# microsoft/AI2BMD

Hardware: NVIDIA H100
Metric: MD steps/sec (higher is better)
Workload: dtype f32

## Files before the change

ai2bmd_b200/csrc/common.cuh:

```cuda
#pragma once
#include <cuda_runtime.h>
#include <stdint.h>

namespace vb {

constexpr int D = 128;
constexpr int H = 8;
constexpr int NR = 32;
constexpr int L = 6;
constexpr int KNB = 32;
constexpr int LDS_PAD = 4;

__device__ __forceinline__ float sigmoidf_(float x) { return __fdividef(1.0f, 1.0f + __expf(-x)); }
__device__ __forceinline__ float silu_(float x) { return __fdividef(x, 1.0f + __expf(-x)); }
__device__ __forceinline__ float dsilu_(float x) {
    float s = sigmoidf_(x);
    return s * (1.0f + x * (1.0f - s));
}

__device__ __forceinline__ float4 ld4(const float* p) { return *reinterpret_cast<const float4*>(p); }
__device__ __forceinline__ float4 ldg4(const float* p) { return __ldg(reinterpret_cast<const float4*>(p)); }
__device__ __forceinline__ void st4(float* p, float4 v) { *reinterpret_cast<float4*>(p) = v; }
__device__ __forceinline__ void red4(float* p, float4 v) { atomicAdd(reinterpret_cast<float4*>(p), v); }

__device__ __forceinline__ float4 f4(float a, float b, float c, float d) { return make_float4(a, b, c, d); }
__device__ __forceinline__ float4 f4s(float a) { return make_float4(a, a, a, a); }
__device__ __forceinline__ float4 operator+(float4 a, float4 b) { return f4(a.x + b.x, a.y + b.y, a.z + b.z, a.w + b.w); }
__device__ __forceinline__ float4 operator-(float4 a, float4 b) { return f4(a.x - b.x, a.y - b.y, a.z - b.z, a.w - b.w); }
__device__ __forceinline__ float4 operator*(float4 a, float4 b) { return f4(a.x * b.x, a.y * b.y, a.z * b.z, a.w * b.w); }
__device__ __forceinline__ float4 operator*(float4 a, float b) { return f4(a.x * b, a.y * b, a.z * b, a.w * b); }
__device__ __forceinline__ float4 operator*(float b, float4 a) { return f4(a.x * b, a.y * b, a.z * b, a.w * b); }
__device__ __forceinline__ float hsum4(float4 a) { return (a.x + a.y) + (a.z + a.w); }
__device__ __forceinline__ float4 silu4(float4 a) { return f4(silu_(a.x), silu_(a.y), silu_(a.z), silu_(a.w)); }
__device__ __forceinline__ float4 dsilu4(float4 a) { return f4(dsilu_(a.x), dsilu_(a.y), dsilu_(a.z), dsilu_(a.w)); }
__device__ __forceinline__ float4 arr4(const float (&a)[4]) { return f4(a[0], a[1], a[2], a[3]); }

__device__ __forceinline__ float warp_sum(float v) {
#pragma unroll
    for (int o = 16; o > 0; o >>= 1) v += __shfl_xor_sync(0xffffffffu, v, o);
    return v;
}
__device__ __forceinline__ float warp_max(float v) {
#pragma unroll
    for (int o = 16; o > 0; o >>= 1) v = fmaxf(v, __shfl_xor_sync(0xffffffffu, v, o));
    return v;
}
__device__ __forceinline__ float warp_min(float v) {
#pragma unroll
    for (int o = 16; o > 0; o >>= 1) v = fminf(v, __shfl_xor_sync(0xffffffffu, v, o));
    return v;
}
__device__ __forceinline__ float quad_sum(float v) {
    v += __shfl_xor_sync(0xffffffffu, v, 1);
    v += __shfl_xor_sync(0xffffffffu, v, 2);
    return v;
}

template <int R>
__device__ __forceinline__ void warp_gemm_group(float (&acc)[R][4], const float* __restrict__ As, int lda, int k,
                                                const float4 (&w)[4]) {
#pragma unroll
    for (int r = 0; r < R; r++) {
        const float4 a = ld4(As + r * lda + k);
        acc[r][0] = fmaf(a.x, w[0].x, acc[r][0]); acc[r][1] = fmaf(a.x, w[0].y, acc[r][1]);
        acc[r][2] = fmaf(a.x, w[0].z, acc[r][2]); acc[r][3] = fmaf(a.x, w[0].w, acc[r][3]);
        acc[r][0] = fmaf(a.y, w[1].x, acc[r][0]); acc[r][1] = fmaf(a.y, w[1].y, acc[r][1]);
        acc[r][2] = fmaf(a.y, w[1].z, acc[r][2]); acc[r][3] = fmaf(a.y, w[1].w, acc[r][3]);
        acc[r][0] = fmaf(a.z, w[2].x, acc[r][0]); acc[r][1] = fmaf(a.z, w[2].y, acc[r][1]);
        acc[r][2] = fmaf(a.z, w[2].z, acc[r][2]); acc[r][3] = fmaf(a.z, w[2].w, acc[r][3]);
        acc[r][0] = fmaf(a.w, w[3].x, acc[r][0]); acc[r][1] = fmaf(a.w, w[3].y, acc[r][1]);
        acc[r][2] = fmaf(a.w, w[3].z, acc[r][2]); acc[r][3] = fmaf(a.w, w[3].w, acc[r][3]);
    }
}
__device__ __forceinline__ void warp_gemm_loadw(float4 (&w)[4], const float* __restrict__ Wp, int ldw, int k) {
    w[0] = ldg4(Wp + (size_t)(k + 0) * ldw);
    w[1] = ldg4(Wp + (size_t)(k + 1) * ldw);
    w[2] = ldg4(Wp + (size_t)(k + 2) * ldw);
    w[3] = ldg4(Wp + (size_t)(k + 3) * ldw);
}

template <int R, int K, int LDA, int NBUF = (R <= 4 ? 4 : 2)>
__device__ __forceinline__ void warp_gemm(float (&acc)[R][4], const float* __restrict__ As,
                                          const float* __restrict__ W, int ldw, int lane, int krot = 0) {
    static_assert(K % 16 == 0, "K must be a multiple of 16");
    const float* Wp = W + lane * 4;
    const auto kk = [&](int k) { return (k + krot) & (K - 1 | -(int)((K & (K - 1)) != 0)); };
    if constexpr (NBUF == 4) {
        float4 w0[4], w1[4], w2[4], w3[4];
        warp_gemm_loadw(w0, Wp, ldw, kk(0));
        warp_gemm_loadw(w1, Wp, ldw, kk(4));
        warp_gemm_loadw(w2, Wp, ldw, kk(8));
#pragma unroll 1
        for (int k = 0; k < K; k += 16) {
            warp_gemm_loadw(w3, Wp, ldw, kk(k + 12));
            warp_gemm_group<R>(acc, As, LDA, kk(k), w0);
            if (k + 16 < K) warp_gemm_loadw(w0, Wp, ldw, kk(k + 16));
            warp_gemm_group<R>(acc, As, LDA, kk(k + 4), w1);
            if (k + 16 < K) warp_gemm_loadw(w1, Wp, ldw, kk(k + 20));
            warp_gemm_group<R>(acc, As, LDA, kk(k + 8), w2);
            if (k + 16 < K) warp_gemm_loadw(w2, Wp, ldw, kk(k + 24));
            warp_gemm_group<R>(acc, As, LDA, kk(k + 12), w3);
        }
    } else {
        float4 w0[4], w1[4];
        warp_gemm_loadw(w0, Wp, ldw, kk(0));
#pragma unroll 1
        for (int k = 0; k < K; k += 8) {
            warp_gemm_loadw(w1, Wp, ldw, kk(k + 4));
            warp_gemm_group<R>(acc, As, LDA, kk(k), w0);
            if (k + 8 < K) warp_gemm_loadw(w0, Wp, ldw, kk(k + 8));
            warp_gemm_group<R>(acc, As, LDA, kk(k + 4), w1);
        }
    }
}

template <int K, int NPRE>
struct WarpGemmPre {
    static_assert((K & (K - 1)) == 0 && K % (4 * NPRE) == 0, "K: power of two and a multiple of the ring");
    float4 w[NPRE][4];
    const float* Wp;
    int ldw, krot;
    __device__ __forceinline__ int kk(int k) const { return (k + krot) & (K - 1); }
    __device__ __forceinline__ void prefetch(const float* __restrict__ W, int ldw_, int lane, int krot_) {
        Wp = W + lane * 4; ldw = ldw_; krot = krot_;
#pragma unroll
        for (int g = 0; g < NPRE; g++) warp_gemm_loadw(w[g], Wp, ldw, kk(4 * g));
    }
    template <int R, int LDA>
    __device__ __forceinline__ void run(float (&acc)[R][4], const float* __restrict__ As) {
#pragma unroll 1
        for (int k = 0; k < K; k += 4 * NPRE) {
#pragma unroll
            for (int g = 0; g < NPRE; g++) {
                warp_gemm_group<R>(acc, As, LDA, kk(k + 4 * g), w[g]);
                if (k + 4 * (g + NPRE) < K) warp_gemm_loadw(w[g], Wp, ldw, kk(k + 4 * (g + NPRE)));
            }
        }
    }
};

template <int R, int K, int LDA>
__device__ __forceinline__ void warp_gemm2(float (&acc)[R][2], const float* __restrict__ As,
                                           const float* __restrict__ W, int ldw, int lane) {
    const float* Wp = W + lane * 2;
#pragma unroll 4
    for (int k = 0; k < K; k += 4) {
        const float2 w0 = __ldg(reinterpret_cast<const float2*>(Wp + (size_t)(k + 0) * ldw));
        const float2 w1 = __ldg(reinterpret_cast<const float2*>(Wp + (size_t)(k + 1) * ldw));
        const float2 w2 = __ldg(reinterpret_cast<const float2*>(Wp + (size_t)(k + 2) * ldw));
        const float2 w3 = __ldg(reinterpret_cast<const float2*>(Wp + (size_t)(k + 3) * ldw));
#pragma unroll
        for (int r = 0; r < R; r++) {
            const float4 a = ld4(As + r * LDA + k);
            acc[r][0] = fmaf(a.x, w0.x, acc[r][0]); acc[r][1] = fmaf(a.x, w0.y, acc[r][1]);
            acc[r][0] = fmaf(a.y, w1.x, acc[r][0]); acc[r][1] = fmaf(a.y, w1.y, acc[r][1]);
            acc[r][0] = fmaf(a.z, w2.x, acc[r][0]); acc[r][1] = fmaf(a.z, w2.y, acc[r][1]);
            acc[r][0] = fmaf(a.w, w3.x, acc[r][0]); acc[r][1] = fmaf(a.w, w3.y, acc[r][1]);
        }
    }
}

template <int R>
__device__ __forceinline__ void acc_set_bias(float (&acc)[R][4], const float* __restrict__ b, int lane) {
    const float4 bb = ldg4(b + lane * 4);
#pragma unroll
    for (int r = 0; r < R; r++) { acc[r][0] = bb.x; acc[r][1] = bb.y; acc[r][2] = bb.z; acc[r][3] = bb.w; }
}
template <int R>
__device__ __forceinline__ void acc_zero(float (&acc)[R][4]) {
#pragma unroll
    for (int r = 0; r < R; r++) { acc[r][0] = 0.f; acc[r][1] = 0.f; acc[r][2] = 0.f; acc[r][3] = 0.f; }
}

__device__ __forceinline__ void pdl_entry() {
    asm volatile("griddepcontrol.wait;" ::: "memory");
}

__device__ __forceinline__ float cutoff_fn(float r, float rc) {
    return (r < rc) ? 0.5f * (cosf(r * (3.14159265358979323846f / rc)) + 1.0f) : 0.0f;
}
__device__ __forceinline__ float cutoff_dfn(float r, float rc) {
    const float w = 3.14159265358979323846f / rc;
    return (r < rc) ? -0.5f * w * sinf(r * w) : 0.0f;
}

}
```

ai2bmd_b200/csrc/k_node2.cuh:

```cuda
#pragma once
#include "k_node.cuh"

namespace vb {

template <int NB> struct N2Cfg {
    static constexpr int WARPS = (NB <= 4) ? 16 : 8; static constexpr int THREADS = WARPS * 32;
    static constexpr int KS = (NB <= 4) ? 2 : 1;
};
template <int NB> struct N2Rows { static constexpr int RB = (NB < 8) ? NB : 8; };

template <int NB>
struct NodeFwd2Smem {
    static constexpr int KS = N2Cfg<NB>::KS;
    static constexpr int LDA = D + LDS_PAD;
    static constexpr int LDO = 3 * D + LDS_PAD;
    float xs[NB][LDA];
    float vs[3 * NB][LDA];
    float os[NB][LDO];
    float osp[(NB <= 4) ? 3 : 1][NB][LDO];
    float px[(KS == 2) ? NB : 1][3 * D];
    float pv[(KS == 2) ? 3 * NB : 1][3 * D];
    float pt[(KS == 2) ? 3 * NB : 1][2 * D];
};

template <int NB>
__global__ void __launch_bounds__(N2Cfg<NB>::THREADS) node_fwd2_kernel(NodeArgs a) {
    pdl_entry();
    extern __shared__ __align__(16) float dyn_smem[];
    const ModelW& mw = a.mw;
    const Workspace& ws = a.ws;
    const int k = a.layer, n0 = (int)blockIdx.x * NB;
    unsigned long long* const tl = a.tl;
    const int krot = a.krot ? (int)blockIdx.x * 16 : 0;
#define N2_TL(i) do { if (tl != nullptr && n0 == 0 && (threadIdx.x & 31) == 0) tl[(i) * 16 + (threadIdx.x >> 5)] = (unsigned long long)clock64(); } while (0)
    N2_TL(0);
    constexpr int N2_WARPS = N2Cfg<NB>::WARPS, N2_THREADS = N2Cfg<NB>::THREADS, KS = N2Cfg<NB>::KS;
    using S = NodeFwd2Smem<NB>;
    constexpr int LDA = S::LDA;
    constexpr int N2_RB = N2Rows<NB>::RB;
    S& sm = *reinterpret_cast<S*>(dyn_smem);
    const int lane = threadIdx.x & 31, warp = threadIdx.x >> 5, col = lane * 4;
    const int nn = min(NB, ws.N - n0);

    if (k >= 1) {
        const LayerW& lw = mw.layer[k - 1];
        for (int idx = threadIdx.x; idx < NB * 32; idx += N2_THREADS) {
            const int nd = idx >> 5, c4 = (idx & 31) * 4;
            st4(&sm.xs[nd][c4], nd < nn ? ld4(ws.XA + (size_t)(n0 + nd) * D + c4) : f4s(0.f));
        }
        [[maybe_unused]] WarpGemmPre<D / 4, 4> go;
        if constexpr (KS == 2) {
            if (warp < 12) go.prefetch(lw.WoT + (size_t)(warp / 3) * (D / 4) * 3 * D + (warp % 3) * D, 3 * D, lane, krot);
        }
        __syncthreads();
        N2_TL(1);
        if constexpr (KS == 2) {
            if (warp < 12) {
                const int ch = warp % 3, kq = warp / 3;
                float acc[N2_RB][4];
                if (kq == 0) acc_set_bias<N2_RB>(acc, lw.bo + ch * D, lane);
                else acc_zero<N2_RB>(acc);
                go.template run<N2_RB, LDA>(acc, &sm.xs[0][kq * (D / 4)]);
#pragma unroll
                for (int r = 0; r < N2_RB; r++) {
                    if (kq == 0) st4(&sm.os[r][ch * D + col], arr4(acc[r]));
                    else st4(&sm.osp[kq - 1][r][ch * D + col], arr4(acc[r]));
                }
            }
            N2_TL(2);
            __syncthreads();
            N2_TL(3);
            for (int idx = threadIdx.x; idx < NB * 96; idx += N2_THREADS) {
                const int r = idx / 96, c4 = (idx % 96) * 4;
                st4(&sm.os[r][c4], (ld4(&sm.os[r][c4]) + ld4(&sm.osp[0][r][c4])) + (ld4(&sm.osp[1][r][c4]) + ld4(&sm.osp[2][r][c4])));
            }
        } else if constexpr (NB <= 4) {
            for (int u = warp; u < 12; u += N2_WARPS) {
                const int ch = u % 3, kq = u / 3;
                float acc[N2_RB][4];
                if (kq == 0) acc_set_bias<N2_RB>(acc, lw.bo + ch * D, lane);
                else acc_zero<N2_RB>(acc);
                warp_gemm<N2_RB, D / 4, LDA, 4>(acc, &sm.xs[0][kq * (D / 4)], lw.WoT + (size_t)kq * (D / 4) * 3 * D + ch * D, 3 * D, lane, krot);
#pragma unroll
                for (int r = 0; r < N2_RB; r++) {
                    if (kq == 0) st4(&sm.os[r][ch * D + col], arr4(acc[r]));
                    else st4(&sm.osp[kq - 1][r][ch * D + col], arr4(acc[r]));
                }
            }
            N2_TL(2);
            __syncthreads();
            N2_TL(3);
            for (int idx = threadIdx.x; idx < NB * 96; idx += N2_THREADS) {
                const int r = idx / 96, c4 = (idx % 96) * 4;
                st4(&sm.os[r][c4], (ld4(&sm.os[r][c4]) + ld4(&sm.osp[0][r][c4])) + (ld4(&sm.osp[1][r][c4]) + ld4(&sm.osp[2][r][c4])));
            }
        } else {
            for (int u = warp; u < 3 * (NB / N2_RB); u += N2_WARPS) {
                const int ch = u % 3, rb = u / 3;
                float acc[N2_RB][4];
                acc_set_bias<N2_RB>(acc, lw.bo + ch * D, lane);
                warp_gemm<N2_RB, D, LDA, (NB <= 8 ? 4 : 2)>(acc, &sm.xs[rb * N2_RB][0], lw.WoT + ch * D, 3 * D, lane);
#pragma unroll
                for (int r = 0; r < N2_RB; r++) st4(&sm.os[rb * N2_RB + r][ch * D + col], arr4(acc[r]));
            }
        }
        __syncthreads();
        N2_TL(4);
    }
    for (int nd = warp; nd < NB; nd += N2_WARPS) {
        const int node = n0 + nd;
        const bool ok = nd < nn;
        float4 x = f4s(0.f), vec[3] = {f4s(0.f), f4s(0.f), f4s(0.f)};
        if (k >= 1) {
            if (ok) {
                const float4 o1 = ld4(&sm.os[nd][col]), o2 = ld4(&sm.os[nd][D + col]), o3 = ld4(&sm.os[nd][2 * D + col]);
                float* orow = ws.O[k - 1] + (size_t)node * 3 * D;
                st4(orow + col, o1); st4(orow + D + col, o2); st4(orow + 2 * D + col, o3);
                x = ld4(ws.X[k - 1] + (size_t)node * D + col) + ld4(ws.VDOT[k - 1] + (size_t)node * D + col) * o2 + o3;
                st4(ws.X[k] + (size_t)node * D + col, x);
#pragma unroll
                for (int s = 0; s < 3; s++) {
                    const size_t r3 = (size_t)node * 3 + s;
                    vec[s] = ld4(ws.V[k - 1] + r3 * D + col) + ld4(ws.V123[k - 1] + r3 * 3 * D + 2 * D + col) * o1 +
                             ld4(ws.VA + r3 * D + col);
                    st4(ws.V[k] + r3 * D + col, vec[s]);
                }
            }
        } else if (ok) {
            x = ld4(ws.X[0] + (size_t)node * D + col);
        }
        if (ok) {
            st4(ws.XA + (size_t)node * D + col, f4s(0.f));
#pragma unroll
            for (int s = 0; s < 3; s++) st4(ws.VA + ((size_t)node * 3 + s) * D + col, f4s(0.f));
        }
        if (k < L) {
            const LayerW& lw = mw.layer[k];
            st4(&sm.xs[nd][col], ln_forward(x, lw.ln_w, lw.ln_b, lane));
            float4 vn[3];
            vecln_forward(vec, vn, lw.vln_w, lane);
#pragma unroll
            for (int s = 0; s < 3; s++) {
                st4(&sm.vs[nd * 3 + s][col], vn[s]);
                if (ok) st4(ws.VN[k] + ((size_t)node * 3 + s) * D + col, vn[s]);
            }
        }
    }
    N2_TL(5);
    if (k >= L) return;
    const LayerW& lw = mw.layer[k];
    constexpr int RV = 3 * NB, KH = D / 2;
    [[maybe_unused]] WarpGemmPre<KH, 2> gm;
    [[maybe_unused]] const int nunits2 = (k < L - 1) ? 16 : 12;
    [[maybe_unused]] const int kind = warp < 6 ? 0 : (warp < 12 ? 1 : 2);
    [[maybe_unused]] const int uv = kind == 0 ? warp : (kind == 1 ? warp - 6 : warp - 12);
    [[maybe_unused]] const int ch2 = kind == 2 ? (uv & 1) : uv % 3, half = kind == 2 ? (uv >> 1) : uv / 3;
    [[maybe_unused]] const bool active = warp < nunits2;
    if constexpr (KS == 2) {
        if (active) {
            const float* W = kind == 0 ? lw.WqkvT : (kind == 1 ? lw.WvecT : lw.WtuT);
            const int ldw = kind == 2 ? 2 * D : 3 * D;
            gm.prefetch(W + (size_t)half * KH * ldw + ch2 * D, ldw, lane, krot);
        }
    }
    __syncthreads();
    N2_TL(6);
    if constexpr (KS == 2) {
        const int ch = ch2;
        float acc[RV][4];
        float (&accx)[NB][4] = *reinterpret_cast<float (*)[NB][4]>(&acc[0][0]);
        if (active) {
            if (kind == 0) {
                if (half == 0) acc_set_bias<NB>(accx, lw.bqkv + ch * D, lane);
                else acc_zero<NB>(accx);
                gm.template run<NB, LDA>(accx, &sm.xs[0][half * KH]);
                if (half == 1) {
#pragma unroll
                    for (int r = 0; r < NB; r++) st4(&sm.px[r][ch * D + col], arr4(accx[r]));
                }
            } else {
                acc_zero<RV>(acc);
                gm.template run<RV, LDA>(acc, &sm.vs[0][half * KH]);
                if (half == 1) {
#pragma unroll
                    for (int r = 0; r < RV; r++) {
                        if (kind == 1) st4(&sm.pv[r][ch * D + col], arr4(acc[r]));
                        else           st4(&sm.pt[r][ch * D + col], arr4(acc[r]));
                    }
                }
            }
        }
        N2_TL(7);
        __syncthreads();
        N2_TL(8);
        if (active && half == 0) {
            if (kind == 0) {
#pragma unroll
                for (int r = 0; r < NB; r++)
                    if (r < nn) st4(ws.QKV[k] + (size_t)(n0 + r) * 3 * D + ch * D + col, arr4(accx[r]) + ld4(&sm.px[r][ch * D + col]));
            } else if (kind == 1) {
#pragma unroll
                for (int r = 0; r < RV; r++)
                    if (r / 3 < nn) st4(ws.V123[k] + ((size_t)n0 * 3 + r) * 3 * D + ch * D + col, arr4(acc[r]) + ld4(&sm.pv[r][ch * D + col]));
            } else {
#pragma unroll
                for (int r = 0; r < RV; r++)
                    if (r / 3 < nn) st4(ws.TU[k] + ((size_t)n0 * 3 + r) * 2 * D + ch * D + col, arr4(acc[r]) + ld4(&sm.pt[r][ch * D + col]));
            }
        }
    } else {
        constexpr int UQ = 3 * (NB / N2_RB), UV = 3 * (3 * NB / N2_RB), UT = 2 * (3 * NB / N2_RB);
        const int nunits = UQ + UV + ((k < L - 1) ? UT : 0);
        for (int u = warp; u < nunits; u += N2_WARPS) {
            float acc[N2_RB][4];
            if (u < UQ) {
                const int ch = u % 3, rb = u / 3;
                acc_set_bias<N2_RB>(acc, lw.bqkv + ch * D, lane);
                warp_gemm<N2_RB, D, LDA, (NB <= 8 ? 4 : 2)>(acc, &sm.xs[rb * N2_RB][0], lw.WqkvT + ch * D, 3 * D, lane);
    #pragma unroll
                for (int r = 0; r < N2_RB; r++) {
                    const int nd = rb * N2_RB + r;
                    if (nd < nn) st4(ws.QKV[k] + (size_t)(n0 + nd) * 3 * D + ch * D + col, arr4(acc[r]));
                }
            } else if (u < UQ + UV) {
                const int v = u - UQ, ch = v % 3, rb = v / 3;
                acc_zero<N2_RB>(acc);
                warp_gemm<N2_RB, D, LDA, (NB <= 8 ? 4 : 2)>(acc, &sm.vs[rb * N2_RB][0], lw.WvecT + ch * D, 3 * D, lane);
    #pragma unroll
                for (int r = 0; r < N2_RB; r++) {
                    const int row = rb * N2_RB + r;
                    if (row / 3 < nn) st4(ws.V123[k] + ((size_t)n0 * 3 + row) * 3 * D + ch * D + col, arr4(acc[r]));
                }
            } else {
                const int v = u - UQ - UV, ch = v % 2, rb = v / 2;
                acc_zero<N2_RB>(acc);
                warp_gemm<N2_RB, D, LDA, (NB <= 8 ? 4 : 2)>(acc, &sm.vs[rb * N2_RB][0], lw.WtuT + ch * D, 2 * D, lane);
    #pragma unroll
                for (int r = 0; r < N2_RB; r++) {
                    const int row = rb * N2_RB + r;
                    if (row / 3 < nn) st4(ws.TU[k] + ((size_t)n0 * 3 + row) * 2 * D + ch * D + col, arr4(acc[r]));
                }
            }
        }
    }
    N2_TL(9);
    __syncthreads();
    N2_TL(10);
    for (int nd = warp; nd < nn; nd += N2_WARPS) {
        const size_t r3 = (size_t)(n0 + nd) * 3;
        float4 vd = f4s(0.f);
#pragma unroll
        for (int s = 0; s < 3; s++) vd = vd + ld4(ws.V123[k] + (r3 + s) * 3 * D + col) * ld4(ws.V123[k] + (r3 + s) * 3 * D + D + col);
        st4(ws.VDOT[k] + (size_t)(n0 + nd) * D + col, vd);
    }
    N2_TL(11);
}

template <int NB>
struct NodeBwd2Smem {
    static constexpr int KS = N2Cfg<NB>::KS;
    static constexpr int LD3 = 3 * D + LDS_PAD;
    static constexpr int LD2 = 2 * D + LDS_PAD;
    static constexpr int NVB = 3 * NB / N2Rows<NB>::RB;
    static constexpr int NXB = NB / N2Rows<NB>::RB;
    float gq[NB][LD3];
    float gvp[3 * NB][LD3];
    float gtu[3 * NB][LD2];
    float part_x[3 * KS][NB][D];
    float part_v[5 * KS][3 * NB][D];
};

template <int NB>
__global__ void __launch_bounds__(N2Cfg<NB>::THREADS) node_bwd2_kernel(NodeArgs a) {
    pdl_entry();
    extern __shared__ __align__(16) float dyn_smem[];
    const ModelW& mw = a.mw;
    const Workspace& ws = a.ws;
    const int k = a.layer, n0 = (int)blockIdx.x * NB;
    unsigned long long* const tl = a.tl;
    const int krot = a.krot ? (int)blockIdx.x * 16 : 0;
    float* __restrict__ const GQKV = ws.GQKV;
    float* __restrict__ const GVNMSG = ws.GVNMSG;
    float* __restrict__ const GTU = ws.GTU;
    constexpr int N2_WARPS = N2Cfg<NB>::WARPS, KS = N2Cfg<NB>::KS;
    N2_TL(0);
    using S = NodeBwd2Smem<NB>;
    constexpr int LD3 = S::LD3, LD2 = S::LD2;
    constexpr int N2_RB = N2Rows<NB>::RB;
    S& sm = *reinterpret_cast<S*>(dyn_smem);
    const int lane = threadIdx.x & 31, warp = threadIdx.x >> 5, col = lane * 4;
    const int nn = min(NB, ws.N - n0);
    const bool has_a = (k <= L - 1), has_b = (k >= 1);
    const bool has_tu = (k < L - 1);
    const float4 z4 = f4s(0.f);

    if (has_a) {
        const LayerW& lw = mw.layer[k];
        for (int nd = warp; nd < NB; nd += N2_WARPS) {
            const int node = n0 + nd;
            const bool ok = nd < nn;
            const float4 gx = ok ? ld4(ws.GX + (size_t)node * D + col) : z4;
            const float* orow = ws.O[k] + (size_t)node * 3 * D;
            const float4 o1 = ok ? ld4(orow + col) : z4, o2 = ok ? ld4(orow + D + col) : z4;
            const float4 g_vdot = gx * o2;
            const float* gq = GQKV + (size_t)node * 3 * D;
            st4(&sm.gq[nd][col], ok ? ld4(gq + col) : z4);
            st4(&sm.gq[nd][D + col], ok ? ld4(gq + D + col) : z4);
            st4(&sm.gq[nd][2 * D + col], ok ? ld4(gq + 2 * D + col) : z4);
#pragma unroll
            for (int s = 0; s < 3; s++) {
                const size_t r3 = (size_t)node * 3 + s;
                const float* vrow = ws.V123[k] + r3 * 3 * D;
                const float4 gv = ok ? ld4(ws.GVEC + r3 * D + col) : z4;
                st4(&sm.gvp[nd * 3 + s][col], g_vdot * (ok ? ld4(vrow + D + col) : z4));
                st4(&sm.gvp[nd * 3 + s][D + col], g_vdot * (ok ? ld4(vrow + col) : z4));
                st4(&sm.gvp[nd * 3 + s][2 * D + col], gv * o1);
                if (has_tu) {
                    const float* gt = GTU + r3 * 2 * D;
                    st4(&sm.gtu[nd * 3 + s][col], ok ? ld4(gt + col) : z4);
                    st4(&sm.gtu[nd * 3 + s][D + col], ok ? ld4(gt + D + col) : z4);
                }
            }
        }
        constexpr int RV = 3 * NB, KH = D / 2;
        [[maybe_unused]] WarpGemmPre<KH, 2> gm;
        [[maybe_unused]] const int kv2 = has_tu ? 5 : 3;
        if constexpr (KS == 2) {
            const int u = warp;
            if (u < 6) gm.prefetch(lw.WqkvN + ((size_t)(u >> 1) * D + (u & 1) * KH) * D, D, lane, krot);
            else if (u < 6 + 2 * kv2) {
                const int v = u - 6, kc = v >> 1, hf = v & 1;
                gm.prefetch((kc < 3 ? lw.WvecN + (size_t)kc * D * D : lw.WtuN + (size_t)(kc - 3) * D * D) + (size_t)hf * KH * D, D, lane, krot);
            }
        }
        N2_TL(1);
        __syncthreads();
        N2_TL(2);
        if constexpr (KS == 2) {
            const int u = warp;
            if (u < 6) {
                const int kc = u >> 1, half = u & 1;
                float acc[NB][4];
                acc_zero<NB>(acc);
                gm.template run<NB, LD3>(acc, &sm.gq[0][kc * D + half * KH]);
#pragma unroll
                for (int r = 0; r < NB; r++) st4(&sm.part_x[u][r][col], arr4(acc[r]));
            } else if (u < 6 + 2 * kv2) {
                const int v = u - 6, kc = v >> 1, half = v & 1;
                float acc[RV][4];
                acc_zero<RV>(acc);
                if (kc < 3) gm.template run<RV, LD3>(acc, &sm.gvp[0][kc * D + half * KH]);
                else        gm.template run<RV, LD2>(acc, &sm.gtu[0][(kc - 3) * D + half * KH]);
#pragma unroll
                for (int r = 0; r < RV; r++) st4(&sm.part_v[v][r][col], arr4(acc[r]));
            }
        } else {
            constexpr int UX = 3 * S::NXB;
            const int kv = has_tu ? 5 : 3;
            const int nunits = UX + kv * S::NVB;
            for (int u = warp; u < nunits; u += N2_WARPS) {
                float acc[N2_RB][4];
                acc_zero<N2_RB>(acc);
                if (u < UX) {
                    const int kc = u % 3, rb = u / 3;
                    warp_gemm<N2_RB, D, LD3, 4>(acc, &sm.gq[rb * N2_RB][kc * D], lw.WqkvN + (size_t)kc * D * D, D, lane);
    #pragma unroll
                    for (int r = 0; r < N2_RB; r++) st4(&sm.part_x[kc][rb * N2_RB + r][col], arr4(acc[r]));
                } else {
                    const int v = u - UX, kc = v % kv, rb = v / kv;
                    if (kc < 3) warp_gemm<N2_RB, D, LD3, 4>(acc, &sm.gvp[rb * N2_RB][kc * D], lw.WvecN + (size_t)kc * D * D, D, lane);
                    else        warp_gemm<N2_RB, D, LD2, 4>(acc, &sm.gtu[rb * N2_RB][(kc - 3) * D], lw.WtuN + (size_t)(kc - 3) * D * D, D, lane);
    #pragma unroll
                    for (int r = 0; r < N2_RB; r++) st4(&sm.part_v[kc][rb * N2_RB + r][col], arr4(acc[r]));
                }
            }
        }
        N2_TL(3);
        __syncthreads();
        N2_TL(4);
    }
    for (int nd = warp; nd < NB; nd += N2_WARPS) {
        const int node = n0 + nd;
        const bool ok = nd < nn;
        float4 gx = ok ? ld4(ws.GX + (size_t)node * D + col) : z4, gvec[3];
#pragma unroll
        for (int s = 0; s < 3; s++) gvec[s] = ok ? ld4(ws.GVEC + ((size_t)node * 3 + s) * D + col) : z4;
        float4 v3p[3] = {z4, z4, z4}, vdp = z4;
        if (has_b && ok) {
#pragma unroll
            for (int s = 0; s < 3; s++) v3p[s] = ld4(ws.V123[k - 1] + ((size_t)node * 3 + s) * 3 * D + 2 * D + col);
            vdp = ld4(ws.VDOT[k - 1] + (size_t)node * D + col);
        }
        if (has_a && ok) {
            const LayerW& lw = mw.layer[k];
            const auto px = [&](int kc) {
                if constexpr (KS == 2) return ld4(&sm.part_x[2 * kc][nd][col]) + ld4(&sm.part_x[2 * kc + 1][nd][col]);
                else return ld4(&sm.part_x[kc][nd][col]);
            };
            const float4 gxn = (px(0) + px(1)) + px(2);
            float4 vin[3], gout[3], gv[3];
#pragma unroll
            for (int s = 0; s < 3; s++) {
                const int row = nd * 3 + s;
                const auto pv = [&](int kc) {
                    if constexpr (KS == 2) return ld4(&sm.part_v[2 * kc][row][col]) + ld4(&sm.part_v[2 * kc + 1][row][col]);
                    else return ld4(&sm.part_v[kc][row][col]);
                };
                float4 g = ld4(GVNMSG + ((size_t)node * 3 + s) * D + col);
                g = g + ((pv(0) + pv(1)) + pv(2));
                if (has_tu) g = g + (pv(3) + pv(4));
                gout[s] = g;
                vin[s] = ld4(ws.V[k] + ((size_t)node * 3 + s) * D + col);
            }
            vecln_backward(vin, gout, gv, lw.vln_w, lane);
#pragma unroll
            for (int s = 0; s < 3; s++) gvec[s] = gvec[s] + gv[s];
            gx = gx + ln_backward(ld4(ws.X[k] + (size_t)node * D + col), gxn, lw.ln_w, lane);
        }
        if (ok) {
            float* gq = GQKV + (size_t)node * 3 * D;
            st4(gq + col, z4); st4(gq + D + col, z4); st4(gq + 2 * D + col, z4);
#pragma unroll
            for (int s = 0; s < 3; s++) {
                const size_t r3 = (size_t)node * 3 + s;
                st4(GVNMSG + r3 * D + col, z4);
                st4(GTU + r3 * 2 * D + col, z4);
                st4(GTU + r3 * 2 * D + D + col, z4);
                st4(ws.GVEC + r3 * D + col, gvec[s]);
            }
            st4(ws.GX + (size_t)node * D + col, gx);
        }
        if (has_b) {
            float4 go1 = z4;
#pragma unroll
            for (int s = 0; s < 3; s++) go1 = go1 + gvec[s] * v3p[s];
            __syncwarp();
            st4(&sm.gq[nd][col], go1);
            st4(&sm.gq[nd][D + col], gx * vdp);
            st4(&sm.gq[nd][2 * D + col], gx);
        }
    }
    N2_TL(5);
    if (!has_b) return;
    const LayerW& lwo = mw.layer[k - 1];
    [[maybe_unused]] WarpGemmPre<D / 4, 4> go;
    if constexpr (KS == 2) {
        if (warp < 12) go.prefetch(lwo.WoN + ((size_t)(warp >> 2) * D + (warp & 3) * (D / 4)) * D, D, lane, krot);
    }
    __syncthreads();
    N2_TL(6);
    if constexpr (KS == 2) {
        float (*po)[NB][D] = reinterpret_cast<float (*)[NB][D]>(&sm.part_v[0][0][0]);
        if (warp < 12) {
            const int kc = warp >> 2, q = warp & 3;
            float acc[NB][4];
            acc_zero<NB>(acc);
            go.template run<NB, LD3>(acc, &sm.gq[0][kc * D + q * (D / 4)]);
#pragma unroll
            for (int r = 0; r < NB; r++) st4(&po[warp][r][col], arr4(acc[r]));
        }
        N2_TL(7);
        __syncthreads();
        N2_TL(8);
        for (int nd = warp; nd < nn; nd += N2_WARPS) {
            float4 t[3];
#pragma unroll
            for (int kc = 0; kc < 3; kc++)
                t[kc] = (ld4(&po[4 * kc][nd][col]) + ld4(&po[4 * kc + 1][nd][col])) + (ld4(&po[4 * kc + 2][nd][col]) + ld4(&po[4 * kc + 3][nd][col]));
            st4(ws.GXA + (size_t)(n0 + nd) * D + col, (t[0] + t[1]) + t[2]);
        }
        N2_TL(9);
    } else {
        for (int u = warp; u < 3 * S::NXB; u += N2_WARPS) {
            const int kc = u % 3, rb = u / 3;
            float acc[N2_RB][4];
            acc_zero<N2_RB>(acc);
            warp_gemm<N2_RB, D, LD3, 4>(acc, &sm.gq[rb * N2_RB][kc * D], lwo.WoN + (size_t)kc * D * D, D, lane);
#pragma unroll
            for (int r = 0; r < N2_RB; r++) st4(&sm.part_x[kc][rb * N2_RB + r][col], arr4(acc[r]));
        }
        __syncthreads();
        for (int nd = warp; nd < nn; nd += N2_WARPS)
            st4(ws.GXA + (size_t)(n0 + nd) * D + col,
                (ld4(&sm.part_x[0][nd][col]) + ld4(&sm.part_x[1][nd][col])) + ld4(&sm.part_x[2][nd][col]));
    }
}
#undef N2_TL

}
```

Measured before the change: 1154.

## Prefetch node glue inputs via cp.async and split scalar/vector glue across warps

The forward and backward node kernels now stage their per-node glue inputs (X, VDOT, V, V123, VA, GX, GVEC, GVNMSG and others) into shared memory with cp.async, issued before the weight prefetch and GEMMs. This hides global load latency behind other work. The glue loop is split so scalar and vector parts run on separate warps, and the partial-sum reduction of os/osp is folded into those warps, removing one block barrier. VDOT is computed from registers after a named barrier between two warps instead of re-reading V123 after a full sync. The cost is extra shared memory per block, which may lower occupancy, plus more complex synchronisation, and the NB<=4 path is removed.

```diff
diff --git a/ai2bmd_b200/csrc/common.cuh b/ai2bmd_b200/csrc/common.cuh
--- a/ai2bmd_b200/csrc/common.cuh
+++ b/ai2bmd_b200/csrc/common.cuh
@@ -22,6 +22,10 @@
 __device__ __forceinline__ float4 ldg4(const float* p) { return __ldg(reinterpret_cast<const float4*>(p)); }
 __device__ __forceinline__ void st4(float* p, float4 v) { *reinterpret_cast<float4*>(p) = v; }
 __device__ __forceinline__ void red4(float* p, float4 v) { atomicAdd(reinterpret_cast<float4*>(p), v); }
+__device__ __forceinline__ void cp4(float* s, const float* g) {
+    asm volatile("cp.async.cg.shared.global [%0], [%1], 16;" ::"r"((uint32_t)__cvta_generic_to_shared(s)), "l"(g) : "memory");
+}
+__device__ __forceinline__ void cp4_wait() { asm volatile("cp.async.wait_all;" ::: "memory"); }
 
 __device__ __forceinline__ float4 f4(float a, float b, float c, float d) { return make_float4(a, b, c, d); }
 __device__ __forceinline__ float4 f4s(float a) { return make_float4(a, a, a, a); }
diff --git a/ai2bmd_b200/csrc/k_node2.cuh b/ai2bmd_b200/csrc/k_node2.cuh
--- a/ai2bmd_b200/csrc/k_node2.cuh
+++ b/ai2bmd_b200/csrc/k_node2.cuh
@@ -18,6 +18,8 @@
     float vs[3 * NB][LDA];
     float os[NB][LDO];
     float osp[(NB <= 4) ? 3 : 1][NB][LDO];
+    float gl[(KS == 2) ? 11 * NB : 1][D];
+    float v1[(KS == 2) ? 3 * NB : 1][D];
     float px[(KS == 2) ? NB : 1][3 * D];
     float pv[(KS == 2) ? 3 * NB : 1][3 * D];
     float pt[(KS == 2) ? 3 * NB : 1][2 * D];
@@ -42,16 +44,35 @@
     const int lane = threadIdx.x & 31, warp = threadIdx.x >> 5, col = lane * 4;
     const int nn = min(NB, ws.N - n0);
 
+    [[maybe_unused]] const auto glue_in = [&](int row, const float* g) {
+        if constexpr (KS == 2) return ld4(&sm.gl[row][col]);
+        else return ld4(g + col);
+    };
     if (k >= 1) {
         const LayerW& lw = mw.layer[k - 1];
-        for (int idx = threadIdx.x; idx < NB * 32; idx += N2_THREADS) {
-            const int nd = idx >> 5, c4 = (idx & 31) * 4;
-            st4(&sm.xs[nd][c4], nd < nn ? ld4(ws.XA + (size_t)(n0 + nd) * D + c4) : f4s(0.f));
+        constexpr int NR = (KS == 2) ? 12 * NB : NB;
+        for (int idx = threadIdx.x; idx < NR * 32; idx += N2_THREADS) {
+            const int q = idx >> 5, c4 = (idx & 31) * 4;
+            const float* src;
+            int nd;
+            if (q < NB) { nd = q; src = ws.XA + (size_t)(n0 + nd) * D; }
+            else if (q < 2 * NB) { nd = q - NB; src = ws.X[k - 1] + (size_t)(n0 + nd) * D; }
+            else if (q < 3 * NB) { nd = q - 2 * NB; src = ws.VDOT[k - 1] + (size_t)(n0 + nd) * D; }
+            else {
+                const int r = (q - 3 * NB) % (3 * NB), part = (q - 3 * NB) / (3 * NB);
+                const size_t r3 = (size_t)n0 * 3 + r;
+                nd = r / 3;
+                src = part == 0 ? ws.V[k - 1] + r3 * D : (part == 1 ? ws.V123[k - 1] + r3 * 3 * D + 2 * D : ws.VA + r3 * D);
+            }
+            float* dst = q < NB ? &sm.xs[q][c4] : &sm.gl[q - NB][c4];
+            if (nd < nn) cp4(dst, src + c4);
+            else st4(dst, f4s(0.f));
         }
         [[maybe_unused]] WarpGemmPre<D / 4, 4> go;
         if constexpr (KS == 2) {
             if (warp < 12) go.prefetch(lw.WoT + (size_t)(warp / 3) * (D / 4) * 3 * D + (warp % 3) * D, 3 * D, lane, krot);
         }
+        cp4_wait();
         __syncthreads();
         N2_TL(1);
         if constexpr (KS == 2) {
@@ -67,33 +88,6 @@
                     else st4(&sm.osp[kq - 1][r][ch * D + col], arr4(acc[r]));
                 }
             }
-            N2_TL(2);
-            __syncthreads();
-            N2_TL(3);
-            for (int idx = threadIdx.x; idx < NB * 96; idx += N2_THREADS) {
-                const int r = idx / 96, c4 = (idx % 96) * 4;
-                st4(&sm.os[r][c4], (ld4(&sm.os[r][c4]) + ld4(&sm.osp[0][r][c4])) + (ld4(&sm.osp[1][r][c4]) + ld4(&sm.osp[2][r][c4])));
-            }
-        } else if constexpr (NB <= 4) {
-            for (int u = warp; u < 12; u += N2_WARPS) {
-                const int ch = u % 3, kq = u / 3;
-                float acc[N2_RB][4];
-                if (kq == 0) acc_set_bias<N2_RB>(acc, lw.bo + ch * D, lane);
-                else acc_zero<N2_RB>(acc);
-                warp_gemm<N2_RB, D / 4, LDA, 4>(acc, &sm.xs[0][kq * (D / 4)], lw.WoT + (size_t)kq * (D / 4) * 3 * D + ch * D, 3 * D, lane, krot);
-#pragma unroll
-                for (int r = 0; r < N2_RB; r++) {
-                    if (kq == 0) st4(&sm.os[r][ch * D + col], arr4(acc[r]));
-                    else st4(&sm.osp[kq - 1][r][ch * D + col], arr4(acc[r]));
-                }
-            }
-            N2_TL(2);
-            __syncthreads();
-            N2_TL(3);
-            for (int idx = threadIdx.x; idx < NB * 96; idx += N2_THREADS) {
-                const int r = idx / 96, c4 = (idx % 96) * 4;
-                st4(&sm.os[r][c4], (ld4(&sm.os[r][c4]) + ld4(&sm.osp[0][r][c4])) + (ld4(&sm.osp[1][r][c4]) + ld4(&sm.osp[2][r][c4])));
-            }
         } else {
             for (int u = warp; u < 3 * (NB / N2_RB); u += N2_WARPS) {
                 const int ch = u % 3, rb = u / 3;
@@ -104,51 +98,9 @@
                 for (int r = 0; r < N2_RB; r++) st4(&sm.os[rb * N2_RB + r][ch * D + col], arr4(acc[r]));
             }
         }
-        __syncthreads();
-        N2_TL(4);
-    }
-    for (int nd = warp; nd < NB; nd += N2_WARPS) {
-        const int node = n0 + nd;
-        const bool ok = nd < nn;
-        float4 x = f4s(0.f), vec[3] = {f4s(0.f), f4s(0.f), f4s(0.f)};
-        if (k >= 1) {
-            if (ok) {
-                const float4 o1 = ld4(&sm.os[nd][col]), o2 = ld4(&sm.os[nd][D + col]), o3 = ld4(&sm.os[nd][2 * D + col]);
-                float* orow = ws.O[k - 1] + (size_t)node * 3 * D;
-                st4(orow + col, o1); st4(orow + D + col, o2); st4(orow + 2 * D + col, o3);
-                x = ld4(ws.X[k - 1] + (size_t)node * D + col) + ld4(ws.VDOT[k - 1] + (size_t)node * D + col) * o2 + o3;
-                st4(ws.X[k] + (size_t)node * D + col, x);
-#pragma unroll
-                for (int s = 0; s < 3; s++) {
-                    const size_t r3 = (size_t)node * 3 + s;
-                    vec[s] = ld4(ws.V[k - 1] + r3 * D + col) + ld4(ws.V123[k - 1] + r3 * 3 * D + 2 * D + col) * o1 +
-                             ld4(ws.VA + r3 * D + col);
-                    st4(ws.V[k] + r3 * D + col, vec[s]);
-                }
-            }
-        } else if (ok) {
-            x = ld4(ws.X[0] + (size_t)node * D + col);
-        }
-        if (ok) {
-            st4(ws.XA + (size_t)node * D + col, f4s(0.f));
-#pragma unroll
-            for (int s = 0; s < 3; s++) st4(ws.VA + ((size_t)node * 3 + s) * D + col, f4s(0.f));
-        }
-        if (k < L) {
-            const LayerW& lw = mw.layer[k];
-            st4(&sm.xs[nd][col], ln_forward(x, lw.ln_w, lw.ln_b, lane));
-            float4 vn[3];
-            vecln_forward(vec, vn, lw.vln_w, lane);
-#pragma unroll
-            for (int s = 0; s < 3; s++) {
-                st4(&sm.vs[nd * 3 + s][col], vn[s]);
-                if (ok) st4(ws.VN[k] + ((size_t)node * 3 + s) * D + col, vn[s]);
-            }
-        }
-    }
-    N2_TL(5);
-    if (k >= L) return;
-    const LayerW& lw = mw.layer[k];
+        N2_TL(2);
+        __syncthreads();
+    }
     constexpr int RV = 3 * NB, KH = D / 2;
     [[maybe_unused]] WarpGemmPre<KH, 2> gm;
     [[maybe_unused]] const int nunits2 = (k < L - 1) ? 16 : 12;
@@ -156,12 +108,79 @@
     [[maybe_unused]] const int uv = kind == 0 ? warp : (kind == 1 ? warp - 6 : warp - 12);
     [[maybe_unused]] const int ch2 = kind == 2 ? (uv & 1) : uv % 3, half = kind == 2 ? (uv >> 1) : uv / 3;
     [[maybe_unused]] const bool active = warp < nunits2;
-    if constexpr (KS == 2) {
-        if (active) {
+    [[maybe_unused]] const auto prefetch_units = [&]() {
+        if (k < L && active) {
+            const LayerW& lw = mw.layer[k];
             const float* W = kind == 0 ? lw.WqkvT : (kind == 1 ? lw.WvecT : lw.WtuT);
             const int ldw = kind == 2 ? 2 * D : 3 * D;
             gm.prefetch(W + (size_t)half * KH * ldw + ch2 * D, ldw, lane, krot);
         }
+    };
+    if constexpr (KS == 2) {
+        if (warp >= 2 * NB) prefetch_units();
+    }
+    for (int it = warp; it < 2 * NB; it += N2_WARPS) {
+        const int nd = it % NB, node = n0 + nd;
+        const bool ok = nd < nn;
+        const auto o = [&](int c) {
+            if constexpr (KS == 2)
+                return (ld4(&sm.os[nd][c * D + col]) + ld4(&sm.osp[0][nd][c * D + col])) +
+                       (ld4(&sm.osp[1][nd][c * D + col]) + ld4(&sm.osp[2][nd][c * D + col]));
+            else return ld4(&sm.os[nd][c * D + col]);
+        };
+        if (it < NB) {
+            float4 x = f4s(0.f);
+            if (k >= 1) {
+                if (ok) {
+                    const float4 o2 = o(1), o3 = o(2);
+                    float* orow = ws.O[k - 1] + (size_t)node * 3 * D;
+                    st4(orow + D + col, o2); st4(orow + 2 * D + col, o3);
+                    x = glue_in(nd, ws.X[k - 1] + (size_t)node * D) + glue_in(NB + nd, ws.VDOT[k - 1] + (size_t)node * D) * o2 + o3;
+                    st4(ws.X[k] + (size_t)node * D + col, x);
+                }
+            } else if (ok) {
+                x = ld4(ws.X[0] + (size_t)node * D + col);
+            }
+            if (ok) st4(ws.XA + (size_t)node * D + col, f4s(0.f));
+            if (k < L) {
+                const LayerW& lw = mw.layer[k];
+                st4(&sm.xs[nd][col], ln_forward(x, lw.ln_w, lw.ln_b, lane));
+            }
+        } else {
+            float4 vec[3] = {f4s(0.f), f4s(0.f), f4s(0.f)};
+            if (k >= 1 && ok) {
+                const float4 o1 = o(0);
+                st4(ws.O[k - 1] + (size_t)node * 3 * D + col, o1);
+#pragma unroll
+                for (int s = 0; s < 3; s++) {
+                    const int r = nd * 3 + s;
+                    const size_t r3 = (size_t)node * 3 + s;
+                    vec[s] = glue_in(2 * NB + r, ws.V[k - 1] + r3 * D) + glue_in(5 * NB + r, ws.V123[k - 1] + r3 * 3 * D + 2 * D) * o1 +
+                             glue_in(8 * NB + r, ws.VA + r3 * D);
+                    st4(ws.V[k] + r3 * D + col, vec[s]);
+                }
+            }
+            if (ok) {
+#pragma unroll
+                for (int s = 0; s < 3; s++) st4(ws.VA + ((size_t)node * 3 + s) * D + col, f4s(0.f));
+            }
+            if (k < L) {
+                const LayerW& lw = mw.layer[k];
+                float4 vn[3];
+                vecln_forward(vec, vn, lw.vln_w, lane);
+#pragma unroll
+                for (int s = 0; s < 3; s++) {
+                    st4(&sm.vs[nd * 3 + s][col], vn[s]);
+                    if (ok) st4(ws.VN[k] + ((size_t)node * 3 + s) * D + col, vn[s]);
+                }
+            }
+        }
+    }
+    N2_TL(5);
+    if (k >= L) return;
+    const LayerW& lw = mw.layer[k];
+    if constexpr (KS == 2) {
+        if (warp < 2 * NB) prefetch_units();
     }
     __syncthreads();
     N2_TL(6);
@@ -200,8 +219,25 @@
                     if (r < nn) st4(ws.QKV[k] + (size_t)(n0 + r) * 3 * D + ch * D + col, arr4(accx[r]) + ld4(&sm.px[r][ch * D + col]));
             } else if (kind == 1) {
 #pragma unroll
-                for (int r = 0; r < RV; r++)
-                    if (r / 3 < nn) st4(ws.V123[k] + ((size_t)n0 * 3 + r) * 3 * D + ch * D + col, arr4(acc[r]) + ld4(&sm.pv[r][ch * D + col]));
+                for (int r = 0; r < RV; r++) {
+                    const float4 v = arr4(acc[r]) + ld4(&sm.pv[r][ch * D + col]);
+                    if (r / 3 < nn) st4(ws.V123[k] + ((size_t)n0 * 3 + r) * 3 * D + ch * D + col, v);
+                    if (ch == 0) st4(&sm.v1[r][col], v);
+                    acc[r][0] = v.x; acc[r][1] = v.y; acc[r][2] = v.z; acc[r][3] = v.w;
+                }
+                if (ch == 0) {
+                    asm volatile("bar.arrive 1, 64;" ::: "memory");
+                } else if (ch == 1) {
+                    asm volatile("bar.sync 1, 64;" ::: "memory");
+#pragma unroll
+                    for (int nd = 0; nd < NB; nd++) {
+                        if (nd >= nn) break;
+                        float4 vd = f4s(0.f);
+#pragma unroll
+                        for (int s = 0; s < 3; s++) vd = vd + ld4(&sm.v1[nd * 3 + s][col]) * arr4(acc[nd * 3 + s]);
+                        st4(ws.VDOT[k] + (size_t)(n0 + nd) * D + col, vd);
+                    }
+                }
             } else {
 #pragma unroll
                 for (int r = 0; r < RV; r++)
@@ -242,16 +278,15 @@
                 }
             }
         }
-    }
-    N2_TL(9);
-    __syncthreads();
-    N2_TL(10);
-    for (int nd = warp; nd < nn; nd += N2_WARPS) {
-        const size_t r3 = (size_t)(n0 + nd) * 3;
-        float4 vd = f4s(0.f);
-#pragma unroll
-        for (int s = 0; s < 3; s++) vd = vd + ld4(ws.V123[k] + (r3 + s) * 3 * D + col) * ld4(ws.V123[k] + (r3 + s) * 3 * D + D + col);
-        st4(ws.VDOT[k] + (size_t)(n0 + nd) * D + col, vd);
+        N2_TL(9);
+        __syncthreads();
+        for (int nd = warp; nd < nn; nd += N2_WARPS) {
+            const size_t r3 = (size_t)(n0 + nd) * 3;
+            float4 vd = f4s(0.f);
+#pragma unroll
+            for (int s = 0; s < 3; s++) vd = vd + ld4(ws.V123[k] + (r3 + s) * 3 * D + col) * ld4(ws.V123[k] + (r3 + s) * 3 * D + D + col);
+            st4(ws.VDOT[k] + (size_t)(n0 + nd) * D + col, vd);
+        }
     }
     N2_TL(11);
 }
@@ -266,6 +301,7 @@
     float gq[NB][LD3];
     float gvp[3 * NB][LD3];
     float gtu[3 * NB][LD2];
+    float gl[(KS == 2) ? 15 * NB : 1][D];
     float part_x[3 * KS][NB][D];
     float part_v[5 * KS][3 * NB][D];
 };
@@ -282,7 +318,7 @@
     float* __restrict__ const GQKV = ws.GQKV;
     float* __restrict__ const GVNMSG = ws.GVNMSG;
     float* __restrict__ const GTU = ws.GTU;
-    constexpr int N2_WARPS = N2Cfg<NB>::WARPS, KS = N2Cfg<NB>::KS;
+    constexpr int N2_WARPS = N2Cfg<NB>::WARPS, N2_THREADS = N2Cfg<NB>::THREADS, KS = N2Cfg<NB>::KS;
     N2_TL(0);
     using S = NodeBwd2Smem<NB>;
     constexpr int LD3 = S::LD3, LD2 = S::LD2;
@@ -295,36 +331,37 @@
     const float4 z4 = f4s(0.f);
 
     if (has_a) {
+        for (int idx = threadIdx.x; idx < (has_tu ? 9 : 3) * NB * 32; idx += N2_THREADS) {
+            const int q = idx >> 5, c4 = (idx & 31) * 4;
+            int nd;
+            float* dst;
+            const float* src;
+            if (q < 3 * NB) { nd = q / 3; dst = &sm.gq[nd][(q % 3) * D + c4]; src = GQKV + ((size_t)n0 * 3 + q) * D + c4; }
+            else { const int g = q - 3 * NB; nd = g / 6; dst = &sm.gtu[g >> 1][(g & 1) * D + c4]; src = GTU + ((size_t)n0 * 6 + g) * D + c4; }
+            if (nd < nn) cp4(dst, src);
+            else st4(dst, z4);
+        }
+    }
+    if constexpr (KS == 2) {
+        for (int idx = threadIdx.x; idx < 15 * NB * 32; idx += N2_THREADS) {
+            const int q = idx >> 5, c4 = (idx & 31) * 4;
+            int nd;
+            const float* src = nullptr;
+            if (q < NB) { nd = q; src = ws.GX + (size_t)(n0 + nd) * D; }
+            else if (q < 4 * NB) { const int r = q - NB; nd = r / 3; src = ws.GVEC + ((size_t)n0 * 3 + r) * D; }
+            else if (q < 7 * NB) { const int r = q - 4 * NB; nd = r / 3; if (has_b) src = ws.V123[k - 1] + ((size_t)n0 * 3 + r) * 3 * D + 2 * D; }
+            else if (q < 8 * NB) { nd = q - 7 * NB; if (has_b) src = ws.VDOT[k - 1] + (size_t)(n0 + nd) * D; }
+            else if (q < 11 * NB) { const int r = q - 8 * NB; nd = r / 3; if (has_a) src = GVNMSG + ((size_t)n0 * 3 + r) * D; }
+            else if (q < 14 * NB) { const int r = q - 11 * NB; nd = r / 3; if (has_a) src = ws.V[k] + ((size_t)n0 * 3 + r) * D; }
+            else { nd = q - 14 * NB; if (has_a) src = ws.X[k] + (size_t)(n0 + nd) * D; }
+            if (src != nullptr && nd < nn) cp4(&sm.gl[q][c4], src + c4);
+        }
+    }
+    constexpr int RV = 3 * NB, KH = D / 2;
+    [[maybe_unused]] WarpGemmPre<KH, 2> gm;
+    [[maybe_unused]] const int kv2 = has_tu ? 5 : 3;
+    if (has_a) {
         const LayerW& lw = mw.layer[k];
-        for (int nd = warp; nd < NB; nd += N2_WARPS) {
-            const int node = n0 + nd;
-            const bool ok = nd < nn;
-            const float4 gx = ok ? ld4(ws.GX + (size_t)node * D + col) : z4;
-            const float* orow = ws.O[k] + (size_t)node * 3 * D;
-            const float4 o1 = ok ? ld4(orow + col) : z4, o2 = ok ? ld4(orow + D + col) : z4;
-            const float4 g_vdot = gx * o2;
-            const float* gq = GQKV + (size_t)node * 3 * D;
-            st4(&sm.gq[nd][col], ok ? ld4(gq + col) : z4);
-            st4(&sm.gq[nd][D + col], ok ? ld4(gq + D + col) : z4);
-            st4(&sm.gq[nd][2 * D + col], ok ? ld4(gq + 2 * D + col) : z4);
-#pragma unroll
-            for (int s = 0; s < 3; s++) {
-                const size_t r3 = (size_t)node * 3 + s;
-                const float* vrow = ws.V123[k] + r3 * 3 * D;
-                const float4 gv = ok ? ld4(ws.GVEC + r3 * D + col) : z4;
-                st4(&sm.gvp[nd * 3 + s][col], g_vdot * (ok ? ld4(vrow + D + col) : z4));
-                st4(&sm.gvp[nd * 3 + s][D + col], g_vdot * (ok ? ld4(vrow + col) : z4));
-                st4(&sm.gvp[nd * 3 + s][2 * D + col], gv * o1);
-                if (has_tu) {
-                    const float* gt = GTU + r3 * 2 * D;
-                    st4(&sm.gtu[nd * 3 + s][col], ok ? ld4(gt + col) : z4);
-                    st4(&sm.gtu[nd * 3 + s][D + col], ok ? ld4(gt + D + col) : z4);
-                }
-            }
-        }
-        constexpr int RV = 3 * NB, KH = D / 2;
-        [[maybe_unused]] WarpGemmPre<KH, 2> gm;
-        [[maybe_unused]] const int kv2 = has_tu ? 5 : 3;
         if constexpr (KS == 2) {
             const int u = warp;
             if (u < 6) gm.prefetch(lw.WqkvN + ((size_t)(u >> 1) * D + (u & 1) * KH) * D, D, lane, krot);
@@ -333,9 +370,39 @@
                 gm.prefetch((kc < 3 ? lw.WvecN + (size_t)kc * D * D : lw.WtuN + (size_t)(kc - 3) * D * D) + (size_t)hf * KH * D, D, lane, krot);
             }
         }
-        N2_TL(1);
-        __syncthreads();
-        N2_TL(2);
+        constexpr int NP = 9 * NB * 32, PI = (NP + N2_THREADS - 1) / N2_THREADS < 3 ? (NP + N2_THREADS - 1) / N2_THREADS : 3;
+        for (int base = threadIdx.x; base < NP; base += PI * N2_THREADS) {
+            float4 pa[PI], pb[PI], pc[PI];
+#pragma unroll
+            for (int i = 0; i < PI; i++) {
+                const int idx = base + i * N2_THREADS, r = (idx >> 5) / 3, ch = (idx >> 5) % 3, nd = r / 3;
+                pa[i] = z4; pb[i] = z4; pc[i] = z4;
+                if (idx < NP && nd < nn) {
+                    const size_t r3 = (size_t)n0 * 3 + r;
+                    const float* orow = ws.O[k] + (size_t)(n0 + nd) * 3 * D;
+                    if (ch < 2) {
+                        pa[i] = ld4(ws.GX + (size_t)(n0 + nd) * D + col);
+                        pb[i] = ld4(orow + D + col);
+                        pc[i] = ld4(ws.V123[k] + r3 * 3 * D + (1 - ch) * D + col);
+                    } else {
+                        pa[i] = ld4(ws.GVEC + r3 * D + col);
+                        pb[i] = ld4(orow + col);
+                    }
+                }
+            }
+#pragma unroll
+            for (int i = 0; i < PI; i++) {
+                const int idx = base + i * N2_THREADS, r = (idx >> 5) / 3, ch = (idx >> 5) % 3;
+                if (idx < NP) st4(&sm.gvp[r][ch * D + col], ch < 2 ? (pa[i] * pb[i]) * pc[i] : pa[i] * pb[i]);
+            }
+        }
+    }
+    cp4_wait();
+    N2_TL(1);
+    __syncthreads();
+    N2_TL(2);
+    if (has_a) {
+        const LayerW& lw = mw.layer[k];
         if constexpr (KS == 2) {
             const int u = warp;
             if (u < 6) {
@@ -379,65 +446,80 @@
         __syncthreads();
         N2_TL(4);
     }
-    for (int nd = warp; nd < NB; nd += N2_WARPS) {
-        const int node = n0 + nd;
+    [[maybe_unused]] const auto glue_in = [&](int row, const float* g) {
+        if constexpr (KS == 2) return ld4(&sm.gl[row][col]);
+        else return ld4(g + col);
+    };
+    for (int it = warp; it < 2 * NB; it += N2_WARPS) {
+        const int nd = it % NB, node = n0 + nd;
         const bool ok = nd < nn;
-        float4 gx = ok ? ld4(ws.GX + (size_t)node * D + col) : z4, gvec[3];
-#pragma unroll
-        for (int s = 0; s < 3; s++) gvec[s] = ok ? ld4(ws.GVEC + ((size_t)node * 3 + s) * D + col) : z4;
-        float4 v3p[3] = {z4, z4, z4}, vdp = z4;
-        if (has_b && ok) {
-#pragma unroll
-            for (int s = 0; s < 3; s++) v3p[s] = ld4(ws.V123[k - 1] + ((size_t)node * 3 + s) * 3 * D + 2 * D + col);
-            vdp = ld4(ws.VDOT[k - 1] + (size_t)node * D + col);
-        }
-        if (has_a && ok) {
-            const LayerW& lw = mw.layer[k];
-            const auto px = [&](int kc) {
-                if constexpr (KS == 2) return ld4(&sm.part_x[2 * kc][nd][col]) + ld4(&sm.part_x[2 * kc + 1][nd][col]);
-                else return ld4(&sm.part_x[kc][nd][col]);
-            };
-            const float4 gxn = (px(0) + px(1)) + px(2);
-            float4 vin[3], gout[3], gv[3];
+        if (it < NB) {
+            float4 gx = ok ? glue_in(nd, ws.GX + (size_t)node * D) : z4, vdp = z4;
+            if (has_b && ok) vdp = glue_in(7 * NB + nd, ws.VDOT[k - 1] + (size_t)node * D);
+            if (has_a && ok) {
+                const LayerW& lw = mw.layer[k];
+                const auto px = [&](int kc) {
+                    if constexpr (KS == 2) return ld4(&sm.part_x[2 * kc][nd][col]) + ld4(&sm.part_x[2 * kc + 1][nd][col]);
+                    else return ld4(&sm.part_x[kc][nd][col]);
+                };
+                const float4 gxn = (px(0) + px(1)) + px(2);
+                gx = gx + ln_backward(glue_in(14 * NB + nd, ws.X[k] + (size_t)node * D), gxn, lw.ln_w, lane);
+            }
+            if (ok) {
+                float* gq = GQKV + (size_t)node * 3 * D;
+                st4(gq + col, z4); st4(gq + D + col, z4); st4(gq + 2 * D + col, z4);
+                st4(ws.GX + (size_t)node * D + col, gx);
+            }
+            if (has_b) {
+                st4(&sm.gq[nd][D + col], gx * vdp);
+                st4(&sm.gq[nd][2 * D + col], gx);
+            }
+        } else {
+            float4 gvec[3], v3p[3] = {z4, z4, z4};
 #pragma unroll
             for (int s = 0; s < 3; s++) {
                 const int row = nd * 3 + s;
-                const auto pv = [&](int kc) {
-                    if constexpr (KS == 2) return ld4(&sm.part_v[2 * kc][row][col]) + ld4(&sm.part_v[2 * kc + 1][row][col]);
-                    else return ld4(&sm.part_v[kc][row][col]);
-                };
-                float4 g = ld4(GVNMSG + ((size_t)node * 3 + s) * D + col);
-                g = g + ((pv(0) + pv(1)) + pv(2));
-                if (has_tu) g = g + (pv(3) + pv(4));
-                gout[s] = g;
-                vin[s] = ld4(ws.V[k] + ((size_t)node * 3 + s) * D + col);
-            }
-            vecln_backward(vin, gout, gv, lw.vln_w, lane);
-#pragma unroll
-            for (int s = 0; s < 3; s++) gvec[s] = gvec[s] + gv[s];
-            gx = gx + ln_backward(ld4(ws.X[k] + (size_t)node * D + col), gxn, lw.ln_w, lane);
-        }
-        if (ok) {
-            float* gq = GQKV + (size_t)node * 3 * D;
-            st4(gq + col, z4); st4(gq + D + col, z4); st4(gq + 2 * D + col, z4);
-#pragma unroll
-            for (int s = 0; s < 3; s++) {
                 const size_t r3 = (size_t)node * 3 + s;
-                st4(GVNMSG + r3 * D + col, z4);
-                st4(GTU + r3 * 2 * D + col, z4);
-                st4(GTU + r3 * 2 * D + D + col, z4);
-                st4(ws.GVEC + r3 * D + col, gvec[s]);
-            }
-            st4(ws.GX + (size_t)node * D + col, gx);
-        }
-        if (has_b) {
-            float4 go1 = z4;
-#pragma unroll
-            for (int s = 0; s < 3; s++) go1 = go1 + gvec[s] * v3p[s];
-            __syncwarp();
-            st4(&sm.gq[nd][col], go1);
-            st4(&sm.gq[nd][D + col], gx * vdp);
-            st4(&sm.gq[nd][2 * D + col], gx);
+                gvec[s] = ok ? glue_in(NB + row, ws.GVEC + r3 * D) : z4;
+                if (has_b && ok) v3p[s] = glue_in(4 * NB + row, ws.V123[k - 1] + r3 * 3 * D + 2 * D);
+            }
+            if (has_a && ok) {
+                const LayerW& lw = mw.layer[k];
+                float4 vin[3], gout[3], gv[3];
+#pragma unroll
+                for (int s = 0; s < 3; s++) {
+                    const int row = nd * 3 + s;
+                    const size_t r3 = (size_t)node * 3 + s;
+                    const auto pv = [&](int kc) {
+                        if constexpr (KS == 2) return ld4(&sm.part_v[2 * kc][row][col]) + ld4(&sm.part_v[2 * kc + 1][row][col]);
+                        else return ld4(&sm.part_v[kc][row][col]);
+                    };
+                    float4 g = glue_in(8 * NB + row, GVNMSG + r3 * D);
+                    g = g + ((pv(0) + pv(1)) + pv(2));
+                    if (has_tu) g = g + (pv(3) + pv(4));
+                    gout[s] = g;
+                    vin[s] = glue_in(11 * NB + row, ws.V[k] + r3 * D);
+                }
+                vecln_backward(vin, gout, gv, lw.vln_w, lane);
+#pragma unroll
+                for (int s = 0; s < 3; s++) gvec[s] = gvec[s] + gv[s];
+            }
+            if (ok) {
+#pragma unroll
+                for (int s = 0; s < 3; s++) {
+                    const size_t r3 = (size_t)node * 3 + s;
+                    st4(GVNMSG + r3 * D + col, z4);
+                    st4(GTU + r3 * 2 * D + col, z4);
+                    st4(GTU + r3 * 2 * D + D + col, z4);
+                    st4(ws.GVEC + r3 * D + col, gvec[s]);
+                }
+            }
+            if (has_b) {
+                float4 go1 = z4;
+#pragma unroll
+                for (int s = 0; s < 3; s++) go1 = go1 + gvec[s] * v3p[s];
+                st4(&sm.gq[nd][col], go1);
+            }
         }
     }
     N2_TL(5);
```

After: 1170 (median of 6 runs). +1.3%, better.
